# LiqunZhao/Neural-ordinary-differential-equations-based-Lyapunov-Barrier-Actor-Critic-NLBAC

Hardware: AMD Instinct MI355X
Metric: ODE-integrate+update samples/sec, Unicycle batch 4096 (higher is better)
Workload: dtype f32; 1 GPU; Unicycle B=4096 dopri5 (BASELINE.json configs[1] at B=4096 dopri5); NODE fit on 32768 rows every 10 updates; replay of 65536 synthetic transitions resident in HBM; solver=dopri5, adjoint=False, batch_per_gpu=4096, global_batch=4096, node_fit_rows_per_gpu=32768, parallelism=dp1, hipgraph=False

## Files before the change

### neural-ordinary-differential-equations-based-lyapunov-barrier-actor-critic-nlbac_amd/csrc/node_kernels.hip

```cpp
#include "node_rk_shared.h"

#ifdef EXP_TIMING
#define TSTAMP(slot_) if (L.err && blockIdx.x == 0 && tid == 0) reinterpret_cast<long long*>(L.err)[slot_] = (long long)__builtin_readcyclecounter();
#else
#define TSTAMP(slot_)
#endif
template <int MODE, int BITS, int OCC>
__global__ __launch_bounds__(512, OCC ? 4 : 2) void node_rk_fwd_kernel(const NodeRkLaunch L) {
    extern __shared__ __attribute__((aligned(16))) float smem[];
    const int tid = threadIdx.x, t = tid & 255;
    const int grp = __builtin_amdgcn_readfirstlane(tid >> 8);
    const int lane = t & 63, wave = t >> 6;
    __shared__ unsigned s_gcnt[2];
    if (tid < 2) s_gcnt[tid] = 0u;
    GroupBar gbar{&s_gcnt[grp], 0u, 4u};
#ifdef EXP_PRIO
    if (grp == 0) __builtin_amdgcn_s_setprio(EXP_PRIO);
#endif
    const int n = L.n, ns = L.n_s, nu = L.n_u, LD = L.ld;
    const int row0 = blockIdx.x * NLBAC_MLP_TILE;
    const int p_tile = row0 / L.rpp;
    long soff = 0;
    bool fsal = false;
    if (L.ctl) {
// ... 460 lines not shown
        }
#undef has_data
}

__global__ __launch_bounds__(256) void node_du_only_kernel(const float* __restrict__ G, const float* __restrict__ dK,
                                                           int n, int ns, int nu, float* __restrict__ du, int du_acc) {
    const int i = blockIdx.x * 256 + threadIdx.x;
    if (i >= n * nu) return;
    const int row = i / nu, c = i - row * nu;
    float a = 0.f;
    for (int r = 0; r < ns; ++r) a += G[(long)row * ns * nu + r * nu + c] * dK[(long)row * ns + r];
    const float old = du_acc ? du[i] : 0.f;
    du[i] = old + 1.0f * a;
}

extern "C" int nlbac_node_rk_bwd(const nlbac_mlp* f, const nlbac_mlp* g, const float* u, const float* G, int P,
                                 int rows_per_problem, int n_stages_total, int st_lo, int st_hi, int dx_stage0,
                                 const float* beta, const float* h_host, const double* h_dev, int h_dev_stride,
                                 const float* acts_f, long acts_f_ls, const float* acts_g, long acts_g_ls,
                                 int acts_bits, float* dz_f, float* dz_g, float* dG, float* dK, const float* dYup,
                                 float* dy0, int dy0_in, float* du, int du_acc, const nlbac_rk_chain* chain,
                                 int back_idx, nlbac_stream_t s) {
    NLBAC_REQUIRE(f && g && u && G && acts_f && acts_g && dK, "nlbac_node_rk_bwd: null pointer");
    NLBAC_REQUIRE(!(acts_bits && dz_f), "nlbac_node_rk_bwd: weight gradients need the activations, not bit masks");
    NLBAC_REQUIRE(P >= 1 && P <= 8 && rows_per_problem >= 1, "nlbac_node_rk_bwd: bad problem sizes");
    NLBAC_REQUIRE(n_stages_total >= 1 && n_stages_total <= RK_MAX_STAGES && st_lo >= 0 && st_lo < st_hi &&
                      st_hi <= n_stages_total, "nlbac_node_rk_bwd: bad stage range");
    NLBAC_REQUIRE(f->in_dim == g->in_dim && f->in_dim <= RK_MAX_NS && f->out_dim == f->in_dim &&
                      g->out_dim % f->in_dim == 0 && g->out_dim / f->in_dim <= RK_MAX_NU && g->out_dim <= 16,
                  "nlbac_node_rk_bwd: f/g shapes are not a supported control-affine field");
    NLBAC_REQUIRE(f->hid % 4 == 0 && g->hid % 4 == 0 && f->hid <= 256 && g->hid <= 256, "nlbac_node_rk_bwd: bad hid");
#if !defined(EXP_TIMING) && !defined(EXP_TIMING_BWD)
    NLBAC_REQUIRE((dz_f == nullptr) == (dz_g == nullptr) && (dz_f == nullptr) == (dG == nullptr),
                  "nlbac_node_rk_bwd: dz_f, dz_g and dG go together");
#endif
    NLBAC_REQUIRE(h_dev || h_host || (chain && chain->hslots), "nlbac_node_rk_bwd: no step size");
    if (!(chain && chain->ctl) && st_lo == 0 && st_hi == 1 && !dx_stage0 && !dz_f) {
        if (du) {
            const int n = P * rows_per_problem, nu = g->out_dim / f->in_dim;
            hipLaunchKernelGGL(node_du_only_kernel, dim3(nlbac_ceil_div((long)n * nu, 256)), dim3(256), 0, (hipStream_t)s, G, dK, n,
                               f->in_dim, nu, du, du_acc);
            NLBAC_CHECK_LAUNCH("nlbac_node_rk_bwd(du only)");
        }
        return 0;
    }
    NodeRkBwdLaunch L;
    memset(&L, 0, sizeof(L));
// ... 53 lines not shown
    const int mode = (ntf <= 4 && ntg <= 4) ? 1 : ((ntf == 8 && ntg == 8) ? 2 : 0);
    const dim3 grid(nlbac_ceil_div(L.n, NLBAC_MLP_TILE));
    hipLaunchKernelGGL(kb[acts_bits ? 1 : 0][mode], grid, dim3(512), lds, (hipStream_t)s, L);
    NLBAC_CHECK_LAUNCH("nlbac_node_rk_bwd");
    return 0;
}

static int rk_fwd_fill(NodeRkLaunch& L, const nlbac_mlp* f, const nlbac_mlp* g, const float* y0, const float* u, int P,
                       int rows_per_problem, int stage_begin, int stage_end, int n_stages_total, const float* beta,
                       const float* c_out, int n_out, const float* c_err, int n_err, const float* h_host,
                       const double* h_dev, int h_dev_stride, float* K, float* Y, float* G, float* acts_f,
                       long acts_f_ls, float* acts_g, long acts_g_ls, int acts_bits, float* out, float* err,
                       const nlbac_rk_chain* chain, const nlbac_in_map* in_map) {
    NLBAC_REQUIRE(f && g && y0 && u && K && Y && G, "nlbac_node_rk_fwd: null pointer");
    NLBAC_REQUIRE(P >= 1 && P <= 8 && rows_per_problem >= 1, "nlbac_node_rk_fwd: bad problem sizes");
    NLBAC_REQUIRE(n_stages_total >= 1 && n_stages_total <= RK_MAX_STAGES && stage_begin >= 0 &&
                      stage_begin < stage_end && stage_end <= n_stages_total, "nlbac_node_rk_fwd: bad stage range");
    NLBAC_REQUIRE(f->in_dim == g->in_dim && f->in_dim <= RK_MAX_NS && f->out_dim == f->in_dim &&
                      g->out_dim % f->in_dim == 0 && g->out_dim / f->in_dim <= RK_MAX_NU &&
                      g->out_dim <= RK_MAX_GOUT, "nlbac_node_rk_fwd: f/g shapes are not a control-affine field");
    NLBAC_REQUIRE(f->hid % 4 == 0 && g->hid % 4 == 0 && f->hid <= 256 && g->hid <= 256, "nlbac_node_rk_fwd: bad hid");
    NLBAC_REQUIRE(h_dev || h_host, "nlbac_node_rk_fwd: no step size");
    NLBAC_REQUIRE(n_out <= n_stages_total && n_err <= n_stages_total, "nlbac_node_rk_fwd: bad coefficient counts");
    memset(&L, 0, sizeof(L));
    L.net[0] = *f; L.net[1] = *g;
    L.y0 = y0; L.u = u;
    L.in_kind = 0; L.in_obs = nullptr; L.in_obs_ld = 0; L.in_l = 0.f; L.in_ps = nullptr; L.y0_w = nullptr;
    if (in_map && in_map->kind) {
        NLBAC_REQUIRE(in_map->kind == 1 && f->in_dim == 3 && in_map->obs && in_map->obs_ld >= 4 && stage_begin == 0,
                      "nlbac_node_rk_fwd: in map 1 needs n_s == 3, observation rows and a launch that starts at stage 0");
        L.in_kind = 1; L.in_obs = in_map->obs; L.in_obs_ld = in_map->obs_ld; L.in_l = in_map->l; L.in_ps = in_map->ps;
        L.y0_w = const_cast<float*>(y0);
    }
    L.n = P * rows_per_problem; L.rpp = rows_per_problem;
    L.n_s = f->in_dim; L.n_u = g->out_dim / f->in_dim;
    L.stage_begin = stage_begin; L.stage_end = stage_end; L.S_total = n_stages_total;
    if (beta)
        for (int i = 0; i < n_stages_total; ++i)
            for (int j = 0; j < n_stages_total; ++j) L.beta[i][j] = beta[i * n_stages_total + j];
    for (int j = 0; j < n_out; ++j) L.c_out[j] = c_out[j];
    for (int j = 0; j < n_err; ++j) L.c_err[j] = c_err[j];
    L.n_out = out ? n_out : 0; L.n_err = err ? n_err : 0;
    L.h_dev = h_dev; L.h_stride = h_dev_stride;
    for (int p = 0; p < P; ++p) L.h_val[p] = h_host ? h_host[p] : 0.f;
    L.K = K; L.Y = Y; L.G = G;
    L.acts[0] = acts_f; L.acts[1] = acts_g; L.acts_ls[0] = acts_f_ls; L.acts_ls[1] = acts_g_ls;
// ... 128 lines not shown
```

### neural-ordinary-differential-equations-based-lyapunov-barrier-actor-critic-nlbac_amd/csrc/node_rr_kernels.hip

```cpp
#include "node_rk_shared.h"
#include "rr_device.h"
#include <cstdlib>
#include <type_traits>

__device__ __forceinline__ int rr_out_row(int grp, int hu, int ns, int nu) {
    const int qp = hu >> 2, rp = hu & 3, KS0 = (ns + 3) >> 2;
    if (grp == 0) {
        const int c = 4 * rp + qp;
        return (rp < KS0 && c < ns) ? c : -1;
    }
    const int k0 = rp / nu, u = rp - k0 * nu, c = 4 * k0 + qp;
    return (rp < KS0 * nu && c < ns) ? c * nu + u : -1;
}

#ifdef RR_TIMING
#define RSTAMP(slot_) if (L.err && blockIdx.x == 0 && lane == 0 && half == 0) reinterpret_cast<long long*>(L.err)[grp * 256 + (slot_)] = (long long)__builtin_readcyclecounter();
#else
#define RSTAMP(slot_)
#endif

#define RR_MAX_W 4

#ifdef RR_TIMING
__device__ long long g_bwd_stamps[2 * 256];
#define BWSTAMP(slot_) if (blockIdx.x == 0 && lane == 0 && half == 0) g_bwd_stamps[grp * 256 + (slot_)] = (long long)__builtin_readcyclecounter();
extern "C" int nlbac_debug_bwd_stamps(long long* out) {
    return hipMemcpyFromSymbol(out, HIP_SYMBOL(g_bwd_stamps), sizeof(long long) * 2 * 256) == hipSuccess ? 0 : -1;
}
#else
#define BWSTAMP(slot_)
#endif

template <int NB, int R, int BITS, int SPLIT>
__device__ __forceinline__ void node_rr_fwd_body(const NodeRkLaunch& L) {
    using S = RRShape<NB, R>;
    constexpr int KS = S::KS, HID = S::HID;
    constexpr int TB = NB - 2;
    constexpr int NT = KS - 4 * TB;
    constexpr int MF = rr_split_m<S>();
    using PF = RRPart<S, 0, MF>;
    using PG = RRPart<S, MF, S::NM>;
    extern __shared__ __attribute__((aligned(16))) float smem[];
    const int tid = threadIdx.x, lane = tid & 63;
    const int wave = __builtin_amdgcn_readfirstlane(tid >> 6);
    const int grp = wave >> 1, half = wave & 1;
    const int n = L.n, ns = L.n_s, nu = L.n_u, gout = ns * nu;
    const int row0 = blockIdx.x * NLBAC_MLP_TILE;
    RkFwdWhere w;
    if (!rk_fwd_where(L, row0, w)) return;
    RkFwdTile T;
    T.carve(smem);
    float* const sYin = smem + RkFwdTile::floats();
    float* const sW0 = sYin + NLBAC_MLP_TILE * 8;
    float* const sX = sW0 + 2 * 3 * 8 * 64;
    float* const sF2 = sX + 2 * KS * 64;
    unsigned* const sMw = reinterpret_cast<unsigned*>(sF2 + NLBAC_MLP_TILE * RK_MAX_NS);
    int* const sFlag = reinterpret_cast<int*>(sMw + 2 * 2 * 64);
    const nlbac_mlp& net = L.net[grp];
    const int nw = net.n_layers - 1;
    const int n_rows = min(NLBAC_MLP_TILE, n - row0);
    const int q = lane >> 4, r16 = lane & 15;
    const int m = 16 * half + r16, grow = row0 + m;
    const bool row_ok = grow < n;
    const int KS0 = (ns + 3) >> 2;
    const int KL0 = (ns + 4) >> 2;

    const float* const params = net.params;
    int boff[RR_MAX_W];
#pragma unroll
    for (int l = 0; l < RR_MAX_W; ++l) boff[l] = net.b_off[l];
    float* const acts = L.acts[grp] ? L.acts[grp] + w.soff : nullptr;
    const long acts_ls = L.acts_ls[grp];
    const int stage_end = L.stage_end, S_last = L.S_total - 1;
    const bool quiet = L.norm_mode == 1;

    const __amdgpu_buffer_rsrc_t rs = rr_rsrc(net.packed, net.packed_floats);
    const int voff = lane * 16;
    const int wbase = net.rr_fwd_off * 4;
    RRGemm<S> gemm;
    gemm.prime(rs, voff, wbase);

    if (half == 0) {
        const float* W0 = params + net.w_off[0];
        const float* b0 = params + boff[0];
#pragma unroll
        for (int k0 = 0; k0 < 3; ++k0)
#pragma unroll
            for (int jo = 0; jo < NB; ++jo) {
                const int uo = rr_unit_out(NB, R, jo, r16), col = 4 * k0 + q, uc = max(uo, 0);
                const float vw = W0[uc * ns + min(col, ns - 1)], vb = b0[uc];
                sW0[((grp * 3 + k0) * 8 + jo) * 64 + lane] = (uo < 0 || col > ns) ? 0.f : (col < ns ? vw : vb);
            }
    }
    float wo[KS];
    {
// ... 58 lines not shown
        float bn[RK_MAX_STAGES];
        {
            const int sn = min(st + 1, S_last);
#pragma unroll
            for (int j = 0; j < RK_MAX_STAGES; ++j) bn[j] = L.beta[sn][j];
        }
        const long srow = (long)st * n + grow;
        float Ha[KS], Hb[KS];
        f32x4 acc0[NB], acc[NB], bv[NB], bpre[3];
        unsigned wd = 0u;
        constexpr int G0 = rr_group_first(NB);
        auto prefetch_bias = [&](int l) __attribute__((always_inline)) {
#pragma unroll
            for (int jo = 0; jo < G0; ++jo) bpre[jo] = rr_bias<S>(params + boff[l], jo, q);
        };
        prefetch_bias(1);
        PF partF; PG partG;
        if constexpr (SPLIT != 0) {
            if (grp == 0) partF.prime(rs, voff, curF3);
            else partG.prime(rsF, voff, curF3);
        }

        auto save_layer = [&](int l, const float (&H)[KS]) __attribute__((always_inline)) {
            if (BITS || !acts || !row_ok) return;
            float* rowp = acts + (long)l * acts_ls + srow * HID;
#pragma unroll
            for (int jo = 0; jo < NB; ++jo) {
                f32x4 hv{0.f, 0.f, 0.f, 0.f};
#pragma unroll
                for (int rr = 0; rr < ((jo < NB - 1) ? 4 : R); ++rr) hv[rr] = H[4 * jo + rr];
                rr_row_store<S>(rowp, jo, q, hv);
            }
        };
        auto save_word = [&](int l, unsigned word) __attribute__((always_inline)) {
            if (BITS && acts && row_ok) reinterpret_cast<unsigned*>(acts + (long)l * acts_ls)[srow * 4 + q] = word;
        };
        auto pre_l0 = [&](int ks) __attribute__((always_inline)) {
            const int jo = (ks < 4 * (NB - 1)) ? (ks >> 2) : NB - 1, r = ks - 4 * jo;
            const float h = rr_relu(acc0[jo][r]);
            Ha[ks] = h;
            if (BITS) rr_mask_push(wd, h);
            if (ks == KS - 1) save_word(0, wd);
        };
        auto pre_tail = [&](int lp, float (&H)[KS], int t) __attribute__((always_inline)) {
            if (t >= NT) return;
            const int jo = TB + (t >> 2), r = t & 3;
            const float h = rr_relu(acc[jo][r]);
            H[4 * TB + t] = h;
            if (BITS) rr_mask_push(wd, h);
            if (t == NT - 1) save_word(lp, wd);
        };

        {
            float yv[3], a0[3][NB];
#pragma unroll
            for (int k0 = 0; k0 < 3; ++k0) {
                const int col = 4 * k0 + q;
                yv[k0] = (col < ns) ? sYin[m * 8 + min(col, 7)] : (col == ns ? 1.f : 0.f);
// ... 226 lines not shown
    const int row0 = blockIdx.x * NLBAC_MLP_TILE;
    RkBwdWhere w;
    if (!rk_bwd_where(L, row0, w)) return;
    RkBwdTile T;
    T.carve(smem);
    float* const sWt = smem + RkBwdTile::floats();
    float* const sX = sWt + 2 * 4 * 8 * 64;
    float* const sX2 = sX + 2 * KS * 64;
    int* const sFlag = reinterpret_cast<int*>(sX2 + 2 * 16 * 64);
    const nlbac_mlp& net = L.net[grp];
    const int nw = net.n_layers - 1;
    const int q = lane >> 4, r16 = lane & 15;
    const int m = 16 * half + r16, grow = row0 + m;
    const bool row_ok = grow < n;
    const int growc = min(grow, n - 1);
    const int KS0 = (ns + 3) >> 2;
    const int KSO = (grp == 0) ? KS0 : KS0 * nu;
    const bool keep_dz = L.dz[0] != nullptr;

    const float* const params = net.params;
    const float* const acts = L.acts[grp] + w.soff;
    float* const dz = keep_dz ? L.dz[grp] + w.soff : nullptr;
    const long acts_ls = L.acts_ls[grp];
    const int dx_stage0 = L.dx_stage0;

    const __amdgpu_buffer_rsrc_t rs = rr_rsrc(net.packed, net.packed_floats);
    const int voff = lane * 16;
    const int wbase = net.rr_bwd_off * 4;
    RRGemm<S> gemm;
    const int first_l = (SPLIT != 0 && grp == 0) ? nw - 3 : nw - 2;
    gemm.prime(rs, voff, wbase + first_l * S::LAYER_BYTES);
    const nlbac_mlp& netF = L.net[0];
    const __amdgpu_buffer_rsrc_t rsF = rr_rsrc(netF.packed, netF.packed_floats);
    const int curB3 = netF.rr_bwd_off * 4 + 2 * S::LAYER_BYTES;
    if (SPLIT != 0 && tid < 4) sFlag[tid] = 0;

    if (half == 0) {
        const float* Wl = params + net.w_off[nw];
#pragma unroll
        for (int e = 0; e < 4; ++e) {
            int o = -1;
            if (grp == 0) { const int c = 4 * e + q; if (e < KS0 && c < ns) o = c; }
            else { const int k0 = e / nu, u = e - k0 * nu, c = 4 * k0 + q; if (e < KS0 * nu && c < ns) o = c * nu + u; }
#pragma unroll
            for (int jo = 0; jo < NB; ++jo) {
                const int uo = rr_unit_out(NB, R, jo, r16);
// ... 61 lines not shown
                const float v = (grp == 0) ? dk[e] : dk[e] * uu[e];
                dy[e] = ok ? v : 0.f;
                if (grp != 0 && ok && w.gdG && row_ok) w.gdG[((long)st * n + grow) * gout + c * nu + u] = v;
            }
            if (du_thread) {
                float a = 0.f;
#pragma unroll
                for (int r = 0; r < RK_MAX_NS; ++r) a = (r < ns) ? a + gcur[r] * dkd[r] : a;
                T.sDU[du_m * RK_MAX_NU + du_c] = T.sDU[du_m * RK_MAX_NU + du_c] + 1.0f * a;
            }
        }
        if (!data) continue;
        BWSTAMP(sbw + 1)

        const long srow = (long)st * n + growc;
        float Za[KS], Zb[KS];
        f32x4 acct[NB], acc[NB], zero[NB];
#pragma unroll
        for (int jo = 0; jo < NB; ++jo) zero[jo] = f32x4{0.f, 0.f, 0.f, 0.f};
        unsigned mw = 0u, mwt = 0u;
        f32x4 avA[NB], avB[NB], avt[2];
        auto fetch_masks = [&](int l, f32x4 (&av)[NB]) __attribute__((always_inline)) {
            if (BITS) {
                mw = reinterpret_cast<const unsigned*>(acts + (long)l * acts_ls)[srow * 4 + q];
                mw = row_ok ? mw : 0u;
            }
            else {
                const float* arow = acts + (long)l * acts_ls + srow * HID;
#pragma unroll
                for (int jo = 0; jo < NB; ++jo) av[jo] = rr_row_load<S>(arow, jo, q);
            }
        };
        auto save_dz = [&](int l, const float (&Z)[KS]) __attribute__((always_inline)) {
            if (BITS || !dz || !row_ok) return;
            float* rowp = dz + (long)l * acts_ls + ((long)st * n + grow) * HID;
#pragma unroll
            for (int jo = 0; jo < NB; ++jo) {
                f32x4 zv{0.f, 0.f, 0.f, 0.f};
#pragma unroll
                for (int rr = 0; rr < ((jo < NB - 1) ? 4 : R); ++rr) zv[rr] = Z[4 * jo + rr];
                rr_row_store<S>(rowp, jo, q, zv);
            }
        };
        auto pre_top = [&](int ks) __attribute__((always_inline)) {
            const int jo = (ks < 4 * (NB - 1)) ? (ks >> 2) : NB - 1, r = ks - 4 * jo;
            if (BITS) Za[ks] = rr_mask_gate<KS>(mwt, ks, acct[jo][r]);
            else Za[ks] = (row_ok && avA[jo][r] > 0.f) ? acct[jo][r] : 0.f;
        };
        auto pre_tail = [&](float (&Z)[KS], int t) __attribute__((always_inline)) {
            if (t >= NT) return;
            const int jo = TB + (t >> 2), r = t & 3;
            if (BITS) Z[4 * TB + t] = rr_mask_gate<KS>(mwt, 4 * TB + t, acc[jo][r]);
            else Z[4 * TB + t] = (row_ok && avt[jo - TB][r] > 0.f) ? acc[jo][r] : 0.f;
        };

        fetch_masks(nw - 1, avA);
        if (!BITS) fetch_masks(nw - 2, avB);
// ... 90 lines not shown
                partF.prime(rs, voff, curB3);
                if (BITS) fetch_masks(2, avB);
                partF.run(acc, zero, Za, rs, voff, curB3, [&](int) __attribute__((always_inline)) {},
                          [&](int jo, int r) __attribute__((always_inline)) {
                              if (BITS) Zb[4 * jo + r] = rr_mask_gate<KS>(mw, 4 * jo + r, acc[jo][r]);
                              else Zb[4 * jo + r] = (row_ok && avB[jo][r] > 0.f) ? acc[jo][r] : 0.f;
                          });
                save_dz(3, Za);
                if (!BITS) fetch_masks(1, avA);
                avt[0] = avB[TB]; avt[1] = avB[TB + 1];
                while (__hip_atomic_load(sFlag + 2 + half, __ATOMIC_RELAXED, __HIP_MEMORY_SCOPE_WORKGROUP) != key) __builtin_amdgcn_s_sleep(1);
                asm volatile("" ::: "memory");
#pragma unroll
                for (int k = 0; k < PG::K1; ++k) Zb[k] = sX2[(half * 16 + k) * 64 + lane];
                BWSTAMP(sbw + 3)
                prod(I2{}, Zb, Za, avA, avB);
                prod(I3{}, Za, Zb, avB, avA);
                BWSTAMP(sbw + 4)
                dxl(Zb);
            } else {
                unsigned mwF = 0u;
                f32x4 avF[PG::J1];
                if (BITS) {
                    mwF = reinterpret_cast<const unsigned*>(actsF + 2 * L.acts_ls[0])[srow * 4 + q];
                    mwF = row_ok ? mwF : 0u;
                } else {
                    const float* arow = actsF + 2 * L.acts_ls[0] + srow * HID;
#pragma unroll
                    for (int jo = 0; jo < PG::J1; ++jo) avF[jo] = rr_row_load<S>(arow, jo, q);
                }
                PG partG;
                partG.prime(rsF, voff, curB3);
                while (__hip_atomic_load(sFlag + half, __ATOMIC_RELAXED, __HIP_MEMORY_SCOPE_WORKGROUP) != key) __builtin_amdgcn_s_sleep(1);
                asm volatile("" ::: "memory");
#pragma unroll
                for (int ks = 0; ks < KS; ++ks) Zb[ks] = sX[(half * KS + ks) * 64 + lane];
                partG.run(acc, zero, Zb, rsF, voff, curB3, [&](int) __attribute__((always_inline)) {},
                          [&](int, int) __attribute__((always_inline)) {});
#pragma unroll
                for (int jo = 0; jo < PG::J1; ++jo)
#pragma unroll
                    for (int r = 0; r < 4; ++r) {
                        float v;
                        if (BITS) v = rr_mask_gate<KS>(mwF, 4 * jo + r, acc[jo][r]);
                        else v = (row_ok && avF[jo][r] > 0.f) ? acc[jo][r] : 0.f;
                        sX2[(half * 16 + 4 * jo + r) * 64 + lane] = v;
                    }
// ... 59 lines not shown
    if (f->hid != g->hid || rr_shape_index(f->hid) < 0) return false;
    if (f->n_layers != 5 || g->n_layers != 4) return false;
    if (f->rr_fwd_off < 0 || g->rr_fwd_off < 0 || f->rr_bwd_off < 0 || g->rr_bwd_off < 0) return false;
    const int ns = f->in_dim, nu = g->out_dim / (ns > 0 ? ns : 1);
    if (ns < 1 || ns > RK_MAX_NS || nu < 1 || nu > RK_MAX_NU) return false;
    if (((ns + 3) >> 2) * nu > 4) return false;
    return true;
}

extern "C" int nlbac_node_rk_mask_words(const nlbac_mlp* f, const nlbac_mlp* g, int which) {
    if (nlbac_node_rr_eligible(f, g)) return 4;
    const nlbac_mlp* net = which ? g : f;
    return (net->hid + 31) >> 5;
}

static bool rr_split() {
    static const bool on = [] { const char* e = getenv("NLBAC_NODE_SPLIT"); return !(e && e[0] == '0'); }();
    return on;
}

int nlbac_node_rr_fwd_launch(NodeRkLaunch& L, hipStream_t s) {
    if (!nlbac_node_rr_eligible(&L.net[0], &L.net[1])) return 1;
    using KernelF = void (*)(const NodeRkLaunch);
    static const KernelF kf[2][3][2] = {{{node_rr_fwd_kernel<4, 4, 0, 0>, node_rr_fwd_kernel<4, 4, 1, 0>},
                                         {node_rr_fwd_kernel<7, 1, 0, 0>, node_rr_fwd_kernel<7, 1, 1, 0>},
                                         {node_rr_fwd_kernel<8, 4, 0, 0>, node_rr_fwd_kernel<8, 4, 1, 0>}},
                                        {{node_rr_fwd_kernel<4, 4, 0, 1>, node_rr_fwd_kernel<4, 4, 1, 1>},
                                         {node_rr_fwd_kernel<7, 1, 0, 1>, node_rr_fwd_kernel<7, 1, 1, 1>},
                                         {node_rr_fwd_kernel<8, 4, 0, 1>, node_rr_fwd_kernel<8, 4, 1, 1>}}};
    const size_t lds = (size_t)(RkFwdTile::floats() + NLBAC_MLP_TILE * 8 + 2 * 3 * 8 * 64 +
                                2 * 32 * 64 + NLBAC_MLP_TILE * RK_MAX_NS + 2 * 2 * 64 + 4) * sizeof(float);
    const dim3 grid(nlbac_ceil_div(L.n, NLBAC_MLP_TILE));
    hipLaunchKernelGGL(kf[(rr_split() && L.acts_bits) ? 1 : 0][rr_shape_index(L.net[0].hid)][L.acts_bits ? 1 : 0], grid, dim3(256), lds, s, L);
    NLBAC_CHECK_LAUNCH("nlbac_node_rk_fwd(rr)");
    return 0;
}

int nlbac_node_rr_fwd_begin_launch(NodeRkLaunch& LA, NodeRkLaunch& LB, NodeRkLaunch& LC, hipStream_t s) {
    if (!nlbac_node_rr_eligible(&LA.net[0], &LA.net[1]) || !LA.acts_bits) return 1;
    using Kernel3 = void (*)(const NodeRkLaunch, const NodeRkLaunch, const NodeRkLaunch);
    static const Kernel3 k3[2][3] = {{node_rr_fwd_begin_kernel<4, 4, 0>, node_rr_fwd_begin_kernel<7, 1, 0>, node_rr_fwd_begin_kernel<8, 4, 0>},
                                     {node_rr_fwd_begin_kernel<4, 4, 1>, node_rr_fwd_begin_kernel<7, 1, 1>, node_rr_fwd_begin_kernel<8, 4, 1>}};
    const size_t lds = (size_t)(RkFwdTile::floats() + NLBAC_MLP_TILE * 8 + 2 * 3 * 8 * 64 +
                                2 * 32 * 64 + NLBAC_MLP_TILE * RK_MAX_NS + 2 * 2 * 64 + 4) * sizeof(float);
    const dim3 grid(nlbac_ceil_div(LA.n, NLBAC_MLP_TILE));
    hipLaunchKernelGGL(k3[rr_split() ? 1 : 0][rr_shape_index(LA.net[0].hid)], grid, dim3(256), lds, s, LA, LB, LC);
    NLBAC_CHECK_LAUNCH("nlbac_node_rk_fwd_begin(rr)");
    return 0;
}

int nlbac_node_rr_bwd_launch(NodeRkBwdLaunch& L, hipStream_t s) {
    if (!nlbac_node_rr_eligible(&L.net[0], &L.net[1])) return 1;
    using KernelB = void (*)(const NodeRkBwdLaunch);
    static const KernelB kb[2][3][2] = {{{node_rr_bwd_kernel<4, 4, 0, 0>, node_rr_bwd_kernel<4, 4, 1, 0>},
                                         {node_rr_bwd_kernel<7, 1, 0, 0>, node_rr_bwd_kernel<7, 1, 1, 0>},
                                         {node_rr_bwd_kernel<8, 4, 0, 0>, node_rr_bwd_kernel<8, 4, 1, 0>}},
                                        {{node_rr_bwd_kernel<4, 4, 0, 1>, node_rr_bwd_kernel<4, 4, 1, 1>},
                                         {node_rr_bwd_kernel<7, 1, 0, 1>, node_rr_bwd_kernel<7, 1, 1, 1>},
                                         {node_rr_bwd_kernel<8, 4, 0, 1>, node_rr_bwd_kernel<8, 4, 1, 1>}}};
    const size_t lds = (size_t)(RkBwdTile::floats() + 2 * 4 * 8 * 64 + 2 * 32 * 64 + 2 * 16 * 64 + 4) * sizeof(float);
    const dim3 grid(nlbac_ceil_div(L.n, NLBAC_MLP_TILE));
    hipLaunchKernelGGL(kb[rr_split() ? 1 : 0][rr_shape_index(L.net[0].hid)][L.acts_bits ? 1 : 0], grid, dim3(256), lds, s, L);
    NLBAC_CHECK_LAUNCH("nlbac_node_rk_bwd(rr)");
    return 0;
}
```

### neural-ordinary-differential-equations-based-lyapunov-barrier-actor-critic-nlbac_amd/odeint.py

```python
import os
import ctypes as C

import torch

from . import _lib
from ._lib import fptr
from .arena import bwd_weights, io_array, mlp_array, stream_ptr

DP_BETA = [
    [1 / 5],
    [3 / 40, 9 / 40],
    [44 / 45, -56 / 15, 32 / 9],
    [19372 / 6561, -25360 / 2187, 64448 / 6561, -212 / 729],
    [9017 / 3168, -355 / 33, 46732 / 5247, 49 / 176, -5103 / 18656],
    [35 / 384, 0, 500 / 1113, 125 / 192, -2187 / 6784, 11 / 84],
]
DP_C_ERR = [35 / 384 - 1951 / 21600, 0, 500 / 1113 - 22642 / 50085, 125 / 192 - 451 / 720,
            -2187 / 6784 - -12231 / 42400, 11 / 84 - 649 / 6300, -1. / 60.]

TABLEAU = {
    "euler": dict(beta=[], c_sol=[1.0]),
    "rk4": dict(beta=[[1 / 3], [-1 / 3, 1.0], [1.0, -1.0, 1.0]], c_sol=[1 / 8, 3 / 8, 3 / 8, 1 / 8]),
    "dopri5": dict(beta=DP_BETA, c_sol=None),
    "probe": dict(beta=[[1.0]], c_sol=None),
}


HOST_COPY = os.environ.get("NLBAC_HOST_COPY", "kernel")
CTL_POLL = os.environ.get("NLBAC_CTL_POLL", "1") != "0"
_SEQ = [0]
NORM_DEFER_ATTEMPT = os.environ.get("NLBAC_NORM_DEFER_ATTEMPT", "1") != "0"

class _Carver:

    def __init__(self, flat, device):
        self.flat, self.device, self.k = flat, device, 0

    def zeros(self, *shape, dtype=torch.float32):
        numel = 1
        for d in shape:
            numel *= d
        take = (numel + 3) & ~3
        off, self.k = self.k, self.k + take
        if self.flat is None:
            return torch.empty(0, dtype=dtype)
        assert self.k <= self.flat.numel(), "step slot too small"
        t = self.flat[off:off + numel]
        if dtype != torch.float32:
            t = t.view(dtype)
        return t.view(*shape)


class _SlotPool:

# ... 3 lines not shown
        solver.STEP_WS(solver, cap, S, dry).bwd(solver)
        self.slot_floats = (dry.k + 63) & ~63
        if dry_only:
            return
        self.chunks = [torch.zeros(n_slots, self.slot_floats, dtype=torch.float32, device=solver.device)]
        self.views = {}

    def ws(self, n, idx):
        assert n <= self.cap
        w = self.views.get((n, idx))
        if w is None:
            c, i = divmod(idx, self.n_slots)
            while c >= len(self.chunks):
                self.chunks.append(torch.zeros(self.n_slots, self.slot_floats, dtype=torch.float32,
                                               device=self.solver.device))
            for k in [k for k in self.views if k[0] != n]:
                del self.views[k]
            w = self.views[(n, idx)] = self.solver.STEP_WS(self.solver, n, self.S, _Carver(self.chunks[c][i], self.solver.device))
            w.slot, w.pool = idx, self
        return w


class _StepWS:
    ADOPT = ("K", "Y", "gout", "err", "acts_f", "acts_g")

    def __init__(self, solver, n, S, store):
        dev, ns, nu = solver.device, solver.n_s, solver.n_u
        f, g = solver.f, solver.g
        self.n, self.S = n, S
        self._store = store
        z = self._store.zeros
        self.K = z(S, n, ns)
        self.Y = z(S, n, ns)
        self.fout = z(n, ns)
        self.gout = z(S, n, ns * nu)
        self.bits = bool(solver.fused and not solver.keep_acts)
        if self.bits:
            zi = lambda *s: self._store.zeros(*s, dtype=torch.int32)
            lib = _lib.load()
            self.wf = lib.nlbac_node_rk_mask_words(C.byref(f.desc), C.byref(g.desc), 0)
            self.wg = lib.nlbac_node_rk_mask_words(C.byref(f.desc), C.byref(g.desc), 1)
            self.acts_f = zi(f.n_layers - 1, S * n, self.wf)
            self.acts_g = zi(g.n_layers - 1, S * n, self.wg)
        else:
            self.wf, self.wg = f.hid, g.hid
            self.acts_f = z(f.n_layers - 1, S * n, f.hid)
            self.acts_g = z(g.n_layers - 1, S * n, g.hid)
        self.y1 = z(n, ns)
        self.err = z(n, ns)
        self._bwd = None
        self.io_fwd, self.io_bwd = {}, {}

    def bwd(self, solver):
        if self._bwd is None:
            dev, ns, nu, n, S = solver.device, solver.n_s, solver.n_u, self.n, self.S
            f, g = solver.f, solver.g
            z = self._store.zeros
            self.dK = z(S, n, ns)
            keep = solver.keep_acts or not solver.fused
            self.dG = z(S, n, ns * nu) if keep else None
            self.dz_f = z(f.n_layers - 1, S * n, f.hid) if keep else None
            self.dz_g = z(g.n_layers - 1, S * n, g.hid) if keep else None
            self.dXf = z(n, f.in_dim)
            self.dXg = z(n, g.in_dim)
            self.dy0 = z(n, ns)
            self.dy1 = z(n, ns)
            self._bwd = True
        return self


# ... 28 lines not shown
        return lds <= 160 * 1024 - 64

    MAX_SIZES = 2

    def _touch(self, n):
        order = self.__dict__.setdefault("_n_order", [])
        if n in order:
            order.remove(n)
        order.append(n)
        while len(order) > self.MAX_SIZES:
            old = order.pop(0)
            self._scratch.pop(old, None)
            self.generation += 1
        self._cur_n = n

    @staticmethod
    def _bucket(n):
        return n if n <= 4096 else -(-n // 4096) * 4096

    DEFAULT_SLOTS = 4

    def _pool(self, n, S, min_slots=1):
        pools = self.__dict__.setdefault("_pools", {})
        key = (self._bucket(n), S, self.fused, self.keep_acts)
        pool = pools.get(key)
        dropped = False
        if pool is not None and pool.n_slots < min_slots:
            del pools[key]
            pool, dropped = None, True
        if pool is None:
            buckets = list(dict.fromkeys(k[0] for k in pools))
            if key[0] not in buckets and len(buckets) >= self.MAX_SIZES:
                for k in [k for k in pools if k[0] == buckets[0]]:
                    del pools[k]
                dropped = True
            if dropped:
                self.generation += 1
                if not torch.cuda.is_current_stream_capturing():
                    torch.cuda.empty_cache()
            n_slots = max(min_slots, self.DEFAULT_SLOTS if S == 7 else 1)
            pool = _SlotPool(self, key[0], S, n_slots, dry_only=True)
            if pool.slot_floats * 4 * n_slots > self.MAX_POOL_BYTES:
                raise _lib.NlbacError(
                    "dopri5: %d accepted steps of %d rows need %.0f GiB of step slots (limit %.0f GiB): the field has "
                    "become stiff for back-propagation through the steps — use the adjoint (agent.adjoint = True / "
                    "odeint_adjoint), whose memory does not grow with the step count"
                    % (n_slots, key[0], pool.slot_floats * 4 * n_slots / 2 ** 30, self.MAX_POOL_BYTES / 2 ** 30))
# ... 96 lines not shown
            for i, r in enumerate(rows):
                for j, v in enumerate(r):
                    flat[(i + 1) * S + j] = v
            b = self._coefs[key] = (fptr(*flat), S)
        return b

    def _rk_fused(self, ws, y0, u, P, rpp, method, st0, st1, h_host=None, h_dev=None, c_out=None, out=None,
                  c_err=None, err=None, save_acts=True, chain=None):
        beta, S = self._beta(method)
        f, g = self.f, self.g
        n = P * rpp
        save_acts = save_acts and not self.adjoint
        im = None
        if st0 == 0 and self.ctx.pop("in_map_pending", None):
            m, im = self._in_map, _lib.InMap()
            im.kind, im.obs, im.obs_ld, im.l = m["kind"], m["obs"].data_ptr(), m["obs_ld"], m["l"]
            im.ps = m["ps"].data_ptr() if m["ps"] is not None else None
        _lib.call("nlbac_node_rk_fwd", C.byref(f.desc), C.byref(g.desc), y0.data_ptr(), u.data_ptr(), P, rpp,
                  st0, st1, S, beta, c_out, len(c_out) if c_out is not None else 0,
                  c_err, len(c_err) if c_err is not None else 0,
                  fptr(*h_host) if h_host is not None else None, h_dev, _lib.DOPRI_CTL if h_dev else 0,
                  ws.K.data_ptr(), ws.Y.data_ptr(), ws.gout.data_ptr(),
                  ws.acts_f.data_ptr() if save_acts else None, ws.S * n * ws.wf,
                  ws.acts_g.data_ptr() if save_acts else None, ws.S * n * ws.wg, 1 if ws.bits else 0,
                  out.data_ptr() if out is not None else None, err.data_ptr() if err is not None else None,
                  C.byref(chain) if chain is not None else None, C.byref(im) if im is not None else None, stream_ptr())
        self.nfe += st1 - st0

    def _rk_fused_bwd(self, ws, u, P, rpp, method, first_eval, need_dy0, need_params, h_host, h_dev, h_stride, top_up,
                      du, last, chain=None, back_idx=0):
        beta_arr, _ = self._beta(method)
        f, g, S = self.f, self.g, ws.S
        _lib.call("nlbac_node_rk_bwd", C.byref(f.desc), C.byref(g.desc), u.data_ptr(), ws.gout.data_ptr(), P, rpp,
                  S, 0 if first_eval else 1, S, 1 if need_dy0 else 0, beta_arr, h_host, h_dev, h_stride,
                  ws.acts_f.data_ptr(), S * ws.n * ws.wf, ws.acts_g.data_ptr(), S * ws.n * ws.wg,
                  1 if ws.bits else 0, ws.dz_f.data_ptr() if need_params else None,
                  ws.dz_g.data_ptr() if need_params else None, ws.dG.data_ptr() if need_params else None,
                  ws.dK.data_ptr(), top_up.data_ptr() if top_up is not None else None, ws.dy0.data_ptr(), 1,
                  du.data_ptr() if du is not None else None, 0 if last else 1,
                  C.byref(chain) if chain is not None else None, back_idx, stream_ptr())

    def _combine(self, y0, K, n_k, coef, h, P, rpp, out):
        _lib.call("nlbac_rk_combine", y0.data_ptr() if y0 is not None else None, K.data_ptr(), n_k,
                  fptr(*coef), fptr(*h), None, 0, P, rpp, self.n_s, out.data_ptr(), stream_ptr())

    def forward(self, y0, u, P, rpp, method, dt, atol=1e-7, rtol=1e-5):
        self.forward_begin(y0, u, P, rpp, method, dt, atol, rtol)
        return self.forward_finish()

    def forward_begin(self, y0, u, P, rpp, method, dt, atol=1e-7, rtol=1e-5):
        n = P * rpp
        assert y0.shape == (n, self.n_s) and u.shape == (n, self.n_u)
        if self.row_groups > 1:
            assert rpp % self.row_groups == 0, "row_groups must divide the rows of a problem"
            P, rpp = P * self.row_groups, rpp // self.row_groups
        self._touch(n)
        self.stats["solves"] += 1
        self.ctx = dict(method=method, P=P, rpp=rpp, n=n, u=u, y0=y0, steps=[], t_end=float(dt), atol=atol,
                        rtol=rtol)
# ... 234 lines not shown
        om = _lib.OutMap()
        om.kind, om.l, om.p = m["kind"], m["l"], m["p"].data_ptr()
        return om

    def _out_map_bwd(self, n):
        m = self.__dict__.get("_out_map")
        if m is None or m["dp"] is None or not self.ctx.get("out_mapped"):
            return None
        om = _lib.OutMap()
        om.kind, om.l, om.dp = m["kind"], m["l"], m["dp"].data_ptr()
        om.dp2 = m["dp2"].data_ptr() if m["dp2"] is not None else None
        om.x = self.ctx["out"].data_ptr()
        return om

    def _interp_nets(self):
        return C.byref(self.f.desc), C.byref(self.g.desc)

    def _interp_fold(self):
        on = self._interp_fold_on()
        ok = self.__dict__.get("_interp_ok")
        if ok is None:
            ok = self._interp_ok = bool(_lib.load().nlbac_rk_interp_ok(*self._interp_nets()))
        return on and ok and self.fused

    def _chain_ok(self, P, rpp):
        return bool(self.device_loop and self.fused and (P == 1 or rpp % _lib.MLP_TILE == 0))

    def _chain(self, ws0, pool, P, rpp, norm_mode, read_ctl):
        ctx = self.ctx
        ctl = self._ctl(P)
        nblk = (rpp + _lib.MLP_TILE - 1) // _lib.MLP_TILE
        hs = self._buf("hslots%d" % pool.n_slots, P, pool.n_slots, dtype=torch.float64)
        c = _lib.RkChain()
        c.ctl = ctl.data_ptr() if read_ctl else None
        c.slot_floats, c.n_slots = pool.slot_floats, pool.n_slots
        c.rtol, c.atol, c.t_end = ctx["rtol"], ctx["atol"], ctx["t_end"]
        c.ctl_w, c.hslots = ctl.data_ptr(), hs.data_ptr()
        c.alog, c.alog_cap = self._buf("alog", P, self.ALOG_CAP, 3, dtype=torch.float64).data_ptr(), self.ALOG_CAP
        c.ctl_host = None if (torch.cuda.is_current_stream_capturing() or HOST_COPY == "side") else self._ctl_io(P)[1].data_ptr()
        if (self.comm is not None and self.comm.world > 1) or norm_mode not in self.FUSED_NORM_MODES:
            c.norm_mode = -1
        else:
            c.norm_mode = norm_mode
            c.partials = self._buf("cpart", P, nblk, 2).data_ptr()
            c.tickets = self._buf("ctickets", P, dtype=torch.int32).data_ptr()
        return c
# ... 258 lines not shown
                cur_y0 = ws.Y[6]
                idx += 1
                prev = ws
                ws = self._step_ws(n, S, idx)
                ws.Y[0].copy_(prev.Y[6])
                ws.K[0].copy_(prev.K[6])
            self._dopri_attempt(ws, cur_y0, u, P, rpp)
        raise _lib.NlbacError("dopri5: max_num_steps exceeded")

    def _adopt(self, k, p, c, st):
        ctx = self.ctx
        P, rpp, n, S = ctx["P"], ctx["rpp"], ctx["n"], 7
        rows = slice(p * rpp, (p + 1) * rpp)
        k._touch(rpp)
        k.stats["solves"] += 1
        k.ctx = dict(method="dopri5", P=1, rpp=rpp, n=rpp, u=ctx["u"][rows], y0=ctx["y0"][rows], steps=[],
                     t_end=ctx["t_end"], atol=ctx["atol"], rtol=ctx["rtol"])
        s = stream_ptr()
        kws = []
        for j in range(st["idx"] + 1):
            src, dst = self._step_ws(n, S, j), k._step_ws(rpp, S, j)
            for name in src.ADOPT:
                a, b = getattr(src, name), getattr(dst, name)
                w = a.shape[-1]
                _lib.call("nlbac_copy_blocks", a.data_ptr() + 4 * p * rpp * w, n * w, b.data_ptr(), rpp * w, rpp * w,
                          a.numel() // (n * w), s)
            kws.append(dst)
        _lib.call("nlbac_copy_blocks", self._ctl(P).data_ptr() + 8 * _lib.DOPRI_CTL * p, 2 * _lib.DOPRI_CTL,
                  k._ctl(1).data_ptr(), 2 * _lib.DOPRI_CTL, 2 * _lib.DOPRI_CTL, 1, s)
        k.ctx["ctl_host"] = c[p:p + 1].clone()
        steps = [dict(ws=kws[j], h=[step["h"][p]], first=step["first"]) for j, step in enumerate(st["steps"])]
        return dict(steps=steps, info=[[e[p]] for e in st["info"]], idx=st["idx"], attempt=st["attempt"],
                    cur_y0=kws[st["idx"] - 1].Y[6] if st["idx"] else k.ctx["y0"])

    def _solve_split(self, c, st):
        ctx = self.ctx
        self.stats["split"] += 1
        P, rpp, n = ctx["P"], ctx["rpp"], ctx["n"]
        out = self._out_buf(n)
        kids, info = [], []
        for p in range(P):
            if p not in self._children:
                self._children[p] = type(self)(self.node, self.device)
            k = self._children[p]
            k.comm, k.fused, k.keep_acts = self.comm, self.fused, self.keep_acts
            self._ctl_io(1)
# ... 431 lines not shown
        self._ws, self._scratch = {}, {}
        self.nfe = 0
        self._net_arr, self._coefs, self._children = None, {}, {}
        self.fused = self.net.hid <= 128
        self.keep_acts = True
        self.stats = dict(solves=0, single_step=0, multi_attempt=0, split=0)
        self.comm = None
        self.row_groups = 1
        self.adjoint = False
        self.generation = 0
        self.device_loop = True
        self.norm = node.norm_device() if getattr(node, "normalized", False) else None
        if self.norm is not None and not self.fused:
            raise _lib.NlbacError("a normalised NODE needs the fused step kernels (hidden width <= 128)")

    def _nets(self):
        if self._net_arr is None:
            self._net_arr = mlp_array([self.net.desc])
        return self._net_arr

    def _interp_nets(self):
        return C.byref(self.net.desc), None

    def _begin_persistent(self, ws0, ch, y0, u, P, rpp):
        return False

    def _adj_scratch(self, n, S):
        net, ns, nc = self.net, self.n_s, self.n_u
        return dict(ZS=self._buf("cadj_ZS", n, 2 * ns + nc), Xin=self._buf("cadj_Xin", n, net.in_dim),
                    Ay=self._buf("cadj_Ay", n, ns), f=self._buf("cadj_f", n, ns), dX=self._buf("cadj_dX", n, net.in_dim),
                    acts=self._buf("cadj_acts", net.n_layers - 1, n, net.hid))

    def _adj_fused(self):
        f = self.__dict__.get("adj_fused")
        if f is None:
            f = self.adj_fused = bool(_lib.load().nlbac_concat_adj_step_ok(C.byref(self.net.desc)))
        return f

    def _adj_interp_fold(self):
        return self._adj_fused() and self._interp_fold_on()

    def _adj_step(self, w, u, P, rpp, method, st0, st1, h_host=None, h_dev=None, ctl=None, c_out=None, c_err=None,
                  keep=None, interp=False):
        if self._adj_fused():
            beta, S = self._beta(method)
            k = keep or {}
# ... 276 lines not shown
```

Before: 3.634 million samples/s.

## Add acts mode 2: store activation rows plus ReLU mask words for NODE fit

Adds a third activation-storage mode for the register-resident RK kernels. The forward saves full activation rows, for weight gradients, and also packed ReLU mask words placed in an extra layer slot. The backward reads the compact masks instead of full activation rows when applying the ReLU derivative, which cuts memory reads during the NODE-fit backward pass. The cost is one extra layer slot of storage, more kernel template instantiations, and extra mask-word writes in the forward. The mode is enabled by default through NLBAC_FIT_MASKS when keep_acts is on.

```diff
diff --git a/neural-ordinary-differential-equations-based-lyapunov-barrier-actor-critic-nlbac_amd/csrc/node_kernels.hip b/neural-ordinary-differential-equations-based-lyapunov-barrier-actor-critic-nlbac_amd/csrc/node_kernels.hip
--- a/neural-ordinary-differential-equations-based-lyapunov-barrier-actor-critic-nlbac_amd/csrc/node_kernels.hip
+++ b/neural-ordinary-differential-equations-based-lyapunov-barrier-actor-critic-nlbac_amd/csrc/node_kernels.hip
@@ -506,7 +506,10 @@
                                  float* dy0, int dy0_in, float* du, int du_acc, const nlbac_rk_chain* chain,
                                  int back_idx, nlbac_stream_t s) {
     NLBAC_REQUIRE(f && g && u && G && acts_f && acts_g && dK, "nlbac_node_rk_bwd: null pointer");
-    NLBAC_REQUIRE(!(acts_bits && dz_f), "nlbac_node_rk_bwd: weight gradients need the activations, not bit masks");
+    NLBAC_REQUIRE(acts_bits >= 0 && acts_bits <= 2, "nlbac_node_rk_bwd: acts_bits is 0, 1 or 2");
+    NLBAC_REQUIRE(!(acts_bits == 1 && dz_f), "nlbac_node_rk_bwd: weight gradients need the activations, not bit masks");
+    NLBAC_REQUIRE(acts_bits != 2 || nlbac_node_rr_eligible(f, g),
+                  "nlbac_node_rk_bwd: acts_bits 2 (rows + mask words) needs the register-resident kernels (nlbac_rk_interp_ok)");
     NLBAC_REQUIRE(P >= 1 && P <= 8 && rows_per_problem >= 1, "nlbac_node_rk_bwd: bad problem sizes");
     NLBAC_REQUIRE(n_stages_total >= 1 && n_stages_total <= RK_MAX_STAGES && st_lo >= 0 && st_lo < st_hi &&
                       st_hi <= n_stages_total, "nlbac_node_rk_bwd: bad stage range");
@@ -606,6 +609,9 @@
     NLBAC_REQUIRE(f->hid % 4 == 0 && g->hid % 4 == 0 && f->hid <= 256 && g->hid <= 256, "nlbac_node_rk_fwd: bad hid");
     NLBAC_REQUIRE(h_dev || h_host, "nlbac_node_rk_fwd: no step size");
     NLBAC_REQUIRE(n_out <= n_stages_total && n_err <= n_stages_total, "nlbac_node_rk_fwd: bad coefficient counts");
+    NLBAC_REQUIRE(acts_bits >= 0 && acts_bits <= 2, "nlbac_node_rk_fwd: acts_bits is 0, 1 or 2");
+    NLBAC_REQUIRE(acts_bits != 2 || nlbac_node_rr_eligible(f, g),
+                  "nlbac_node_rk_fwd: acts_bits 2 (rows + mask words) needs the register-resident kernels (nlbac_rk_interp_ok)");
     memset(&L, 0, sizeof(L));
     L.net[0] = *f; L.net[1] = *g;
     L.y0 = y0; L.u = u;
diff --git a/neural-ordinary-differential-equations-based-lyapunov-barrier-actor-critic-nlbac_amd/csrc/node_rr_kernels.hip b/neural-ordinary-differential-equations-based-lyapunov-barrier-actor-critic-nlbac_amd/csrc/node_rr_kernels.hip
--- a/neural-ordinary-differential-equations-based-lyapunov-barrier-actor-critic-nlbac_amd/csrc/node_rr_kernels.hip
+++ b/neural-ordinary-differential-equations-based-lyapunov-barrier-actor-critic-nlbac_amd/csrc/node_rr_kernels.hip
@@ -20,6 +20,12 @@
 #endif
 
 #define RR_MAX_W 4
+
+template <int BITS, int HID>
+__device__ __forceinline__ long rr_word_idx(int l, long ls, int nw, long sn, long srow, int q) {
+    static_assert(4 * RR_MAX_W <= HID, "the mask words of every layer must fit one layer slot of rows");
+    return BITS == 2 ? (long)nw * ls + ((long)l * sn + srow) * 4 + q : (long)l * ls + srow * 4 + q;
+}
 
 #ifdef RR_TIMING
 __device__ long long g_bwd_stamps[2 * 256];
@@ -40,6 +46,7 @@
     constexpr int MF = rr_split_m<S>();
     using PF = RRPart<S, 0, MF>;
     using PG = RRPart<S, MF, S::NM>;
+    static_assert(SPLIT == 0 || BITS != 2, "rows + mask words: the forward stays unsplit (see nlbac_node_rr_fwd_launch)");
     extern __shared__ __attribute__((aligned(16))) float smem[];
     const int tid = threadIdx.x, lane = tid & 63;
     const int wave = __builtin_amdgcn_readfirstlane(tid >> 6);
@@ -71,6 +78,7 @@
     for (int l = 0; l < RR_MAX_W; ++l) boff[l] = net.b_off[l];
     float* const acts = L.acts[grp] ? L.acts[grp] + w.soff : nullptr;
     const long acts_ls = L.acts_ls[grp];
+    const long sn = (long)L.S_total * n;
     const int stage_end = L.stage_end, S_last = L.S_total - 1;
     const bool quiet = L.norm_mode == 1;
 
@@ -175,7 +183,7 @@
         }
 
         auto save_layer = [&](int l, const float (&H)[KS]) __attribute__((always_inline)) {
-            if (BITS || !acts || !row_ok) return;
+            if (BITS == 1 || !acts || !row_ok) return;
             float* rowp = acts + (long)l * acts_ls + srow * HID;
 #pragma unroll
             for (int jo = 0; jo < NB; ++jo) {
@@ -185,8 +193,9 @@
                 rr_row_store<S>(rowp, jo, q, hv);
             }
         };
+        constexpr unsigned WMASK = KS >= 32 ? ~0u : (1u << (KS & 31)) - 1u;
         auto save_word = [&](int l, unsigned word) __attribute__((always_inline)) {
-            if (BITS && acts && row_ok) reinterpret_cast<unsigned*>(acts + (long)l * acts_ls)[srow * 4 + q] = word;
+            if (BITS && acts && row_ok) reinterpret_cast<unsigned*>(acts)[rr_word_idx<BITS, HID>(l, acts_ls, nw, sn, srow, q)] = word & WMASK;
         };
         auto pre_l0 = [&](int ks) __attribute__((always_inline)) {
             const int jo = (ks < 4 * (NB - 1)) ? (ks >> 2) : NB - 1, r = ks - 4 * jo;
@@ -459,6 +468,7 @@
     const float* const acts = L.acts[grp] + w.soff;
     float* const dz = keep_dz ? L.dz[grp] + w.soff : nullptr;
     const long acts_ls = L.acts_ls[grp];
+    const long sn = (long)L.S_total * n;
     const int dx_stage0 = L.dx_stage0;
 
     const __amdgpu_buffer_rsrc_t rs = rr_rsrc(net.packed, net.packed_floats);
@@ -566,7 +576,7 @@
         f32x4 avA[NB], avB[NB], avt[2];
         auto fetch_masks = [&](int l, f32x4 (&av)[NB]) __attribute__((always_inline)) {
             if (BITS) {
-                mw = reinterpret_cast<const unsigned*>(acts + (long)l * acts_ls)[srow * 4 + q];
+                mw = reinterpret_cast<const unsigned*>(acts)[rr_word_idx<BITS, HID>(l, acts_ls, nw, sn, srow, q)];
                 mw = row_ok ? mw : 0u;
             }
             else {
@@ -576,7 +586,7 @@
             }
         };
         auto save_dz = [&](int l, const float (&Z)[KS]) __attribute__((always_inline)) {
-            if (BITS || !dz || !row_ok) return;
+            if (BITS == 1 || !dz || !row_ok) return;
             float* rowp = dz + (long)l * acts_ls + ((long)st * n + grow) * HID;
 #pragma unroll
             for (int jo = 0; jo < NB; ++jo) {
@@ -713,7 +723,7 @@
                 unsigned mwF = 0u;
                 f32x4 avF[PG::J1];
                 if (BITS) {
-                    mwF = reinterpret_cast<const unsigned*>(actsF + 2 * L.acts_ls[0])[srow * 4 + q];
+                    mwF = reinterpret_cast<const unsigned*>(actsF)[rr_word_idx<BITS, HID>(2, L.acts_ls[0], netF.n_layers - 1, sn, srow, q)];
                     mwF = row_ok ? mwF : 0u;
                 } else {
                     const float* arow = actsF + 2 * L.acts_ls[0] + srow * HID;
@@ -819,16 +829,16 @@
 int nlbac_node_rr_fwd_launch(NodeRkLaunch& L, hipStream_t s) {
     if (!nlbac_node_rr_eligible(&L.net[0], &L.net[1])) return 1;
     using KernelF = void (*)(const NodeRkLaunch);
-    static const KernelF kf[2][3][2] = {{{node_rr_fwd_kernel<4, 4, 0, 0>, node_rr_fwd_kernel<4, 4, 1, 0>},
-                                         {node_rr_fwd_kernel<7, 1, 0, 0>, node_rr_fwd_kernel<7, 1, 1, 0>},
-                                         {node_rr_fwd_kernel<8, 4, 0, 0>, node_rr_fwd_kernel<8, 4, 1, 0>}},
-                                        {{node_rr_fwd_kernel<4, 4, 0, 1>, node_rr_fwd_kernel<4, 4, 1, 1>},
-                                         {node_rr_fwd_kernel<7, 1, 0, 1>, node_rr_fwd_kernel<7, 1, 1, 1>},
-                                         {node_rr_fwd_kernel<8, 4, 0, 1>, node_rr_fwd_kernel<8, 4, 1, 1>}}};
+    static const KernelF kf[3][3] = {{node_rr_fwd_kernel<4, 4, 0, 0>, node_rr_fwd_kernel<4, 4, 1, 0>, node_rr_fwd_kernel<4, 4, 2, 0>},
+                                     {node_rr_fwd_kernel<7, 1, 0, 0>, node_rr_fwd_kernel<7, 1, 1, 0>, node_rr_fwd_kernel<7, 1, 2, 0>},
+                                     {node_rr_fwd_kernel<8, 4, 0, 0>, node_rr_fwd_kernel<8, 4, 1, 0>, node_rr_fwd_kernel<8, 4, 2, 0>}};
+    static const KernelF kf_split[3] = {node_rr_fwd_kernel<4, 4, 1, 1>, node_rr_fwd_kernel<7, 1, 1, 1>, node_rr_fwd_kernel<8, 4, 1, 1>};
     const size_t lds = (size_t)(RkFwdTile::floats() + NLBAC_MLP_TILE * 8 + 2 * 3 * 8 * 64 +
                                 2 * 32 * 64 + NLBAC_MLP_TILE * RK_MAX_NS + 2 * 2 * 64 + 4) * sizeof(float);
     const dim3 grid(nlbac_ceil_div(L.n, NLBAC_MLP_TILE));
-    hipLaunchKernelGGL(kf[(rr_split() && L.acts_bits) ? 1 : 0][rr_shape_index(L.net[0].hid)][L.acts_bits ? 1 : 0], grid, dim3(256), lds, s, L);
+    const int shape = rr_shape_index(L.net[0].hid);
+    const KernelF k = (rr_split() && L.acts_bits == 1) ? kf_split[shape] : kf[shape][L.acts_bits];
+    hipLaunchKernelGGL(k, grid, dim3(256), lds, s, L);
     NLBAC_CHECK_LAUNCH("nlbac_node_rk_fwd(rr)");
     return 0;
 }
@@ -849,15 +859,16 @@
 int nlbac_node_rr_bwd_launch(NodeRkBwdLaunch& L, hipStream_t s) {
     if (!nlbac_node_rr_eligible(&L.net[0], &L.net[1])) return 1;
     using KernelB = void (*)(const NodeRkBwdLaunch);
-    static const KernelB kb[2][3][2] = {{{node_rr_bwd_kernel<4, 4, 0, 0>, node_rr_bwd_kernel<4, 4, 1, 0>},
-                                         {node_rr_bwd_kernel<7, 1, 0, 0>, node_rr_bwd_kernel<7, 1, 1, 0>},
-                                         {node_rr_bwd_kernel<8, 4, 0, 0>, node_rr_bwd_kernel<8, 4, 1, 0>}},
-                                        {{node_rr_bwd_kernel<4, 4, 0, 1>, node_rr_bwd_kernel<4, 4, 1, 1>},
-                                         {node_rr_bwd_kernel<7, 1, 0, 1>, node_rr_bwd_kernel<7, 1, 1, 1>},
-                                         {node_rr_bwd_kernel<8, 4, 0, 1>, node_rr_bwd_kernel<8, 4, 1, 1>}}};
+    static const KernelB kb[2][3][3] = {
+        {{node_rr_bwd_kernel<4, 4, 0, 0>, node_rr_bwd_kernel<4, 4, 1, 0>, node_rr_bwd_kernel<4, 4, 2, 0>},
+         {node_rr_bwd_kernel<7, 1, 0, 0>, node_rr_bwd_kernel<7, 1, 1, 0>, node_rr_bwd_kernel<7, 1, 2, 0>},
+         {node_rr_bwd_kernel<8, 4, 0, 0>, node_rr_bwd_kernel<8, 4, 1, 0>, node_rr_bwd_kernel<8, 4, 2, 0>}},
+        {{node_rr_bwd_kernel<4, 4, 0, 1>, node_rr_bwd_kernel<4, 4, 1, 1>, node_rr_bwd_kernel<4, 4, 2, 1>},
+         {node_rr_bwd_kernel<7, 1, 0, 1>, node_rr_bwd_kernel<7, 1, 1, 1>, node_rr_bwd_kernel<7, 1, 2, 1>},
+         {node_rr_bwd_kernel<8, 4, 0, 1>, node_rr_bwd_kernel<8, 4, 1, 1>, node_rr_bwd_kernel<8, 4, 2, 1>}}};
     const size_t lds = (size_t)(RkBwdTile::floats() + 2 * 4 * 8 * 64 + 2 * 32 * 64 + 2 * 16 * 64 + 4) * sizeof(float);
     const dim3 grid(nlbac_ceil_div(L.n, NLBAC_MLP_TILE));
-    hipLaunchKernelGGL(kb[rr_split() ? 1 : 0][rr_shape_index(L.net[0].hid)][L.acts_bits ? 1 : 0], grid, dim3(256), lds, s, L);
+    hipLaunchKernelGGL(kb[rr_split() ? 1 : 0][rr_shape_index(L.net[0].hid)][L.acts_bits], grid, dim3(256), lds, s, L);
     NLBAC_CHECK_LAUNCH("nlbac_node_rk_bwd(rr)");
     return 0;
 }
diff --git a/neural-ordinary-differential-equations-based-lyapunov-barrier-actor-critic-nlbac_amd/odeint.py b/neural-ordinary-differential-equations-based-lyapunov-barrier-actor-critic-nlbac_amd/odeint.py
--- a/neural-ordinary-differential-equations-based-lyapunov-barrier-actor-critic-nlbac_amd/odeint.py
+++ b/neural-ordinary-differential-equations-based-lyapunov-barrier-actor-critic-nlbac_amd/odeint.py
@@ -30,6 +30,7 @@
 CTL_POLL = os.environ.get("NLBAC_CTL_POLL", "1") != "0"
 _SEQ = [0]
 NORM_DEFER_ATTEMPT = os.environ.get("NLBAC_NORM_DEFER_ATTEMPT", "1") != "0"
+FIT_MASKS = os.environ.get("NLBAC_FIT_MASKS", "1") != "0"
 
 class _Carver:
 
@@ -79,7 +80,7 @@
 
 
 class _StepWS:
-    ADOPT = ("K", "Y", "gout", "err", "acts_f", "acts_g")
+    ADOPT = ("K", "Y", "gout", "err", "acts_f", "acts_g", "words_f", "words_g")
 
     def __init__(self, solver, n, S, store):
         dev, ns, nu = solver.device, solver.n_s, solver.n_u
@@ -92,6 +93,7 @@
         self.fout = z(n, ns)
         self.gout = z(S, n, ns * nu)
         self.bits = bool(solver.fused and not solver.keep_acts)
+        self.acts_mode = 1 if self.bits else (2 if solver._fit_masks() else 0)
         if self.bits:
             zi = lambda *s: self._store.zeros(*s, dtype=torch.int32)
             lib = _lib.load()
@@ -101,8 +103,18 @@
             self.acts_g = zi(g.n_layers - 1, S * n, self.wg)
         else:
             self.wf, self.wg = f.hid, g.hid
-            self.acts_f = z(f.n_layers - 1, S * n, f.hid)
-            self.acts_g = z(g.n_layers - 1, S * n, g.hid)
+            if self.acts_mode == 2:
+                full_f = z(f.n_layers, S * n, f.hid)
+                full_g = z(g.n_layers, S * n, g.hid)
+                words = lambda t, nw: t[-1].view(-1)[:nw * S * n * 4].view(torch.int32).view(nw, S * n, 4) \
+                    if t.numel() else t
+                self.acts_f, self.words_f = full_f[:-1], words(full_f, f.n_layers - 1)
+                self.acts_g, self.words_g = full_g[:-1], words(full_g, g.n_layers - 1)
+            else:
+                self.acts_f = z(f.n_layers - 1, S * n, f.hid)
+                self.acts_g = z(g.n_layers - 1, S * n, g.hid)
+        if self.acts_mode != 2:
+            self.words_f = self.words_g = None
         self.y1 = z(n, ns)
         self.err = z(n, ns)
         self._bwd = None
@@ -177,7 +189,7 @@
 
     def _pool(self, n, S, min_slots=1):
         pools = self.__dict__.setdefault("_pools", {})
-        key = (self._bucket(n), S, self.fused, self.keep_acts)
+        key = (self._bucket(n), S, self.fused, self.keep_acts, self._fit_masks())
         pool = pools.get(key)
         dropped = False
         if pool is not None and pool.n_slots < min_slots:
@@ -320,7 +332,7 @@
                   fptr(*h_host) if h_host is not None else None, h_dev, _lib.DOPRI_CTL if h_dev else 0,
                   ws.K.data_ptr(), ws.Y.data_ptr(), ws.gout.data_ptr(),
                   ws.acts_f.data_ptr() if save_acts else None, ws.S * n * ws.wf,
-                  ws.acts_g.data_ptr() if save_acts else None, ws.S * n * ws.wg, 1 if ws.bits else 0,
+                  ws.acts_g.data_ptr() if save_acts else None, ws.S * n * ws.wg, ws.acts_mode,
                   out.data_ptr() if out is not None else None, err.data_ptr() if err is not None else None,
                   C.byref(chain) if chain is not None else None, C.byref(im) if im is not None else None, stream_ptr())
         self.nfe += st1 - st0
@@ -332,7 +344,7 @@
         _lib.call("nlbac_node_rk_bwd", C.byref(f.desc), C.byref(g.desc), u.data_ptr(), ws.gout.data_ptr(), P, rpp,
                   S, 0 if first_eval else 1, S, 1 if need_dy0 else 0, beta_arr, h_host, h_dev, h_stride,
                   ws.acts_f.data_ptr(), S * ws.n * ws.wf, ws.acts_g.data_ptr(), S * ws.n * ws.wg,
-                  1 if ws.bits else 0, ws.dz_f.data_ptr() if need_params else None,
+                  ws.acts_mode, ws.dz_f.data_ptr() if need_params else None,
                   ws.dz_g.data_ptr() if need_params else None, ws.dG.data_ptr() if need_params else None,
                   ws.dK.data_ptr(), top_up.data_ptr() if top_up is not None else None, ws.dy0.data_ptr(), 1,
                   du.data_ptr() if du is not None else None, 0 if last else 1,
@@ -613,6 +625,12 @@
         if ok is None:
             ok = self._interp_ok = bool(_lib.load().nlbac_rk_interp_ok(*self._interp_nets()))
         return on and ok and self.fused
+
+    def _fit_masks(self):
+        ok = self.__dict__.get("_interp_ok")
+        if ok is None:
+            ok = self._interp_ok = bool(_lib.load().nlbac_rk_interp_ok(*self._interp_nets()))
+        return bool(FIT_MASKS and ok and self.fused and self.keep_acts)
 
     def _chain_ok(self, P, rpp):
         return bool(self.device_loop and self.fused and (P == 1 or rpp % _lib.MLP_TILE == 0))
@@ -917,6 +935,8 @@
             src, dst = self._step_ws(n, S, j), k._step_ws(rpp, S, j)
             for name in src.ADOPT:
                 a, b = getattr(src, name), getattr(dst, name)
+                if a is None:
+                    continue
                 w = a.shape[-1]
                 _lib.call("nlbac_copy_blocks", a.data_ptr() + 4 * p * rpp * w, n * w, b.data_ptr(), rpp * w, rpp * w,
                           a.numel() // (n * w), s)
@@ -1394,6 +1414,9 @@
     def _interp_nets(self):
         return C.byref(self.net.desc), None
 
+    def _fit_masks(self):
+        return False
+
     def _begin_persistent(self, ws0, ch, y0, u, P, rpp):
         return False
 
```

Measured after the change: 3.676 million samples/s, median of 6. About the same (+1.2%).
